# ml-jku/LaM-SLidE

Measured on AMD Instinct MI355X. Metric: sampled trajectories/sec (50-step ODE) + decoded-coord L2 vs ref, MD17, higher is better.
Workload: dtype bf16; 1 GPU; md17_bench; tail=False, ln_fuse=True, T=30, L=256, C=32, D=512, H=16, depth=4, sampler=ODE, state_updates=50, batch_per_gpu=32, global_batch=32, parallelism=batch-shard x1, 1 gather to rank 0 per step, noise_elem_stride_per_rank=7864320, kernels=general, trajectories_per_pass=32

## Files before the change

lam_slide_amd/csrc/host_launch.hip.h:

```cpp
#pragma once
#include <atomic>
#include <type_traits>

#include "host_common.hip.h"

namespace {

struct HeadArgs {
    float *x, *out;
    const float *h, *shift, *scale;
    int mod_stride;
    const float *Wo, *bo;
    int n, C, tpt, do_step;
    StepUpdate u;
};

#ifdef LSL_EXPERIMENTS
constexpr bool lsl_experiments = true;
template <int NE, int VEC>
bool launch_head_experiment(const HeadArgs &, hipStream_t);
template <class Epi>
bool launch_gemm_experiment(int, const GemmArgs &, const Epi &, hipStream_t, bool);
#else
constexpr bool lsl_experiments = false;
template <int NE, int VEC>
bool launch_head_experiment(const HeadArgs &, hipStream_t) { return false; }
template <class Epi>
bool launch_gemm_experiment(int, const GemmArgs &, const Epi &, hipStream_t, bool) { return false; }
#endif

int env_int(const char *name, int dflt) {
    const char *e = getenv(name);
    return e ? atoi(e) : dflt;
}
int tune_int(const char *name, int dflt) { return lsl_experiments ? env_int(name, dflt) : dflt; }

int device_cus() {
    static std::atomic<int> cache[64];
    int dev = 0;
    if (hipGetDevice(&dev) != hipSuccess) return 256;
    int n = cache[dev & 63].load(std::memory_order_relaxed);
    if (n > 0) return n;
    n = 256;
    (void)hipDeviceGetAttribute(&n, hipDeviceAttributeMultiprocessorCount, dev);
    if (n <= 0) n = 256;
    cache[dev & 63].store(n, std::memory_order_relaxed);
    return n;
}

constexpr size_t LDS_BUDGET = 160 * 1024;


template <int NE, int VEC>
void launch_ln_mod_t(u16 *a, const float *h, const float *shift, const float *scale, int stride, int n, int tpt, hipStream_t st) {
    if constexpr (NE % 4 == 0) {
        static const int persist = tune_int("LSL_LN_PERSIST", 16);
        if (persist > 0) {
            const int grid = std::min((n + 3) / 4, device_cus() * persist);
            static const int nt = (tune_int("LSL_NT", 3) >> 3) & 1;
            hipLaunchKernelGGL((k_ln_modulate_v4<NE>), dim3(grid), dim3(256), 0, st, a, h, shift, scale, stride, n, tpt, nt);
            return;
        }
    }
    hipLaunchKernelGGL((k_ln_modulate<NE, VEC>), dim3((n + 3) / 4), dim3(256), 0, st, a, h, shift, scale, stride, n, tpt);
}
template <int NE, int VEC>
void launch_ln_inplace_t(float *h, int n, float eps, hipStream_t st) {
    hipLaunchKernelGGL((k_ln_inplace<NE, VEC>), dim3((n + 3) / 4), dim3(256), 0, st, h, n, eps);
}
template <int NE, int VEC>
void launch_head_mfma(const HeadArgs &a, hipStream_t st, Profiler *pr = nullptr) {
    if (launch_head_experiment<NE, VEC>(a, st)) return;
    auto kern = k_head_step_mfma<NE, VEC>;
    const size_t lds = head_mfma_lds_bytes<NE>(a.C <= 32);
    LSL_ALLOW_LDS(kern, head_mfma_lds_bytes<NE>(false));
    static const int per_cu = tune_int("LSL_HEAD_PER_CU", 2);
    const int wgs = device_cus() * (per_cu >= 2 && 2 * lds <= LDS_BUDGET ? 2 : 1);
    if (pr) pr->label(4, "k_head_step_mfma<%d, %d> (%s, %d per CU)", NE, VEC, a.C <= 32 ? "one slab" : "cycled slabs", wgs / device_cus());
    hipLaunchKernelGGL(kern, dim3(std::min((a.n + HEAD_TOK - 1) / HEAD_TOK, wgs)), dim3(256), lds, st, a.x, a.out, a.h, a.shift, a.scale, a.mod_stride,
                       a.Wo, a.bo, a.n, a.C, a.tpt, a.do_step, a.u);
}
void launch_state_affine(float *x, unsigned long long n, const StepUpdate &u, hipStream_t st) {
    hipLaunchKernelGGL(k_state_affine, dim3((unsigned)std::min<unsigned long long>((n + 255) / 256, 2048)), dim3(256), 0, st, x, n, u);
}

#define DISPATCH_D(D, FN, ...)                          \
    switch ((D) / 64) {                                 \
        case 1: FN<1, 1>(__VA_ARGS__); break;           \
        case 2: FN<2, 2>(__VA_ARGS__); break;           \
        case 3: FN<3, 1>(__VA_ARGS__); break;           \
        case 4: FN<4, 2>(__VA_ARGS__); break;           \
        case 5: FN<5, 1>(__VA_ARGS__); break;           \
        case 6: FN<6, 2>(__VA_ARGS__); break;           \
        case 7: FN<7, 1>(__VA_ARGS__); break;           \
        default: FN<8, 2>(__VA_ARGS__); break;          \
    }

bool embed_stats_ok(int C, int D) { return C <= 32 && D % 256 == 0 && D <= 512; }
template <int MODE>
int launch_embed(float *out, const float *in, const float *W, const float *b, const float *b2, const float *me,
                 const int64_t *mask, const float *base, int n, int C, int D, hipStream_t st, float2 *stats = nullptr, int npad = 0,
                 Profiler *pr = nullptr) {
    if (C > 32 && C % 8 == 0 && C <= 128 && D % 32 == 0) {
        const int tpw = 3, ngrp = (D / 32 + tpw - 1) / tpw;
        const long units = (long)((n + 31) / 32) * ngrp;
        const dim3 g((unsigned)((units + 3) / 4));
        if (pr) pr->label(5, "k_embed_mfma<%d, %d> (32-token tiles)", MODE, C / 8);
        switch (C / 8) {
#define LSL_EMB_CASE(CK) case CK: hipLaunchKernelGGL((k_embed_mfma<MODE, CK>), g, dim3(256), 0, st, out, in, W, b, b2, me, mask, base, n, C, D, tpw); return 0;
            LSL_EMB_CASE(5) LSL_EMB_CASE(6) LSL_EMB_CASE(7) LSL_EMB_CASE(8) LSL_EMB_CASE(9) LSL_EMB_CASE(10) LSL_EMB_CASE(11) LSL_EMB_CASE(12)
            LSL_EMB_CASE(13) LSL_EMB_CASE(14) LSL_EMB_CASE(15) LSL_EMB_CASE(16)
#undef LSL_EMB_CASE
        }
    }
    int tok = EMB_TOK;
    static const int stage = tune_int("LSL_EMBED_LDS", 1);
    const bool w_lds = stage && C == 32 && D % 4 == 0 && D <= 512;
    if (w_lds)
        while (tok > 16 && (n + tok - 1) / tok < 2 * device_cus()) tok /= 2;
    const dim3 grid(std::min((n + tok - 1) / tok, 2 * device_cus())), blk(256);
    const bool with_stats = stats && MODE == 1 && C <= 32 && embed_stats_ok(C, D);
    if (pr)
        pr->label(5, "k_embed<%d, %d, %d%s> (%d-token tiles%s)", C <= 32 ? 32 : C <= 64 ? 64 : C <= 96 ? 96 : 128, MODE, C <= 32 ? 4 : C <= 96 ? 2 : 1,
                  with_stats ? ", true" : "", tok, w_lds ? ", weights through LDS" : (C & 3) ? ", scalar weight loads" : "");
    if (C <= 32) {
        const size_t lds = w_lds ? embed_w_lds_bytes<32, 4>(D) : 0;
        if (with_stats) {
            auto kern = k_embed<32, 1, 4, true>;
            LSL_ALLOW_LDS(kern, (embed_w_lds_bytes<32, 4>(512)));
            hipLaunchKernelGGL(kern, grid, blk, lds, st, out, in, W, b, b2, me, mask, base, n, C, D, w_lds ? 1 : 0, tok, stats, npad);
            return 0;
        }
        auto kern = k_embed<32, MODE, 4>;
        LSL_ALLOW_LDS(kern, (embed_w_lds_bytes<32, 4>(512)));
        hipLaunchKernelGGL(kern, grid, blk, lds, st, out, in, W, b, b2, me, mask, base, n, C, D, w_lds ? 1 : 0, tok, (float2 *)nullptr, 0);
    } else if (C <= 64) hipLaunchKernelGGL((k_embed<64, MODE, 2>), grid, blk, 0, st, out, in, W, b, b2, me, mask, base, n, C, D, 0, tok, (float2 *)nullptr, 0);
    else if (C <= 96) hipLaunchKernelGGL((k_embed<96, MODE, 2>), grid, blk, 0, st, out, in, W, b, b2, me, mask, base, n, C, D, 0, tok, (float2 *)nullptr, 0);
    else hipLaunchKernelGGL((k_embed<128, MODE, 1>), grid, blk, 0, st, out, in, W, b, b2, me, mask, base, n, C, D, 0, tok, (float2 *)nullptr, 0);
    return 0;
}

template <int BF, int BT, int NWF, int NWT, int BK, int NS, bool PERSIST, class Epi>
void launch_gemm_glds(const GemmArgs &g, const Epi &epi, hipStream_t st) {
    auto kern = k_gemm_glds<BF, BT, NWF, NWT, BK, NS, PERSIST, Epi>;
    const size_t lds = GemmCfg<BF, BT, NWF, NWT, BK, NS, PERSIST, Epi>::lds_bytes + (Epi::lds_bias ? (size_t)((g.F + BF - 1) / BF) * BF * 4 : 0);
    LSL_ALLOW_LDS(kern, LDS_BUDGET);
    const int tiles = ((g.N + BT - 1) / BT) * ((g.F + BF - 1) / BF);
    int grid = tiles;
    if (PERSIST) {
        const int per_cu = (int)std::max<size_t>(1, LDS_BUDGET / lds);
        grid = device_cus() * per_cu;
        grid -= grid % 8;
        if (grid > tiles) grid = tiles;
    }
    hipLaunchKernelGGL(kern, dim3(grid), dim3(NWF * NWT * 64), lds, st, g, epi);
}

}

#ifdef LSL_EXPERIMENTS
#include "host_launch_experiments.hip.h"
#endif

namespace {

template <class Fn>
bool with_linear1_ts_instance(int hdp, int D, Fn &&fn) {
#define X(H, K) if (hdp == H && D == K) return fn(ic<H>{}, ic<K>{}), true;
    LSL_LIN1_TS_INSTANCES(X)
#undef X
    return false;
}
template <int HDP, int K, int NW = 8, bool LNF = false>
void launch_linear1_ts_t(const Lin1Args &a, hipStream_t st) {
    using C = Lin1Cfg<HDP, K, NW>;
    const int ntile = (a.N + C::TT - 1) / C::TT, nb = a.F / 32;
    const long units = (long)ntile * nb;
    int grid = (int)std::min<long>(device_cus(), units / 2);
    Lin1Args b = a;
    static const int align = tune_int("LSL_LIN1_ALIGN", 1);
    const int wpt = std::min(device_cus() / ntile, nb / 2);
    b.wpt = align && wpt >= 2 ? wpt : 0;
    if (b.wpt) grid = b.wpt * ntile;
    lsl_lin1_launch(HDP, K, NW, LNF, b, grid, LNF ? C::lds_bytes_lnf(a.F) : C::lds_bytes(a.F), st);
}
int linear1_ts_waves(int D, int N) {
    static const int nw4_max = tune_int("LSL_LIN1_NW4_MAX", 10240);
    return D == 512 && N <= nw4_max ? 4 : 8;
}
bool linear1_ts_ok(int hdp, int D, int F1, int HHD, int N) {
    static const int on = tune_int("LSL_LIN1_TS", 1);
    if (!on || F1 % 64 != 0 || HHD % 64 != 0 || N < 1) return false;
    size_t lds = 0;
    return with_linear1_ts_instance(hdp, D, [&](auto h, auto k) { lds = Lin1Cfg<decltype(h)::value, decltype(k)::value, 8>::lds_bytes(F1); }) && lds <= LDS_BUDGET;
}
int ln_fuse_env() {
    static const int v = env_int("LSL_LN_FUSE", -1);
    return v;
}
bool linear1_lnf_ok(int hdp, int D, int F1, int HHD, int N, int tpt, int mod_stride) {
    if (ln_fuse_env() == 0 || !linear1_ts_ok(hdp, D, F1, HHD, N)) return false;
    size_t lds = 0;
    int min_tpt = 0;
    with_linear1_ts_instance(hdp, D, [&](auto h, auto k) {
        using C = Lin1Cfg<decltype(h)::value, decltype(k)::value, 8>;
        lds = C::lds_bytes_lnf(F1);
        min_tpt = C::LN_SLOTS >= 3 ? C::TT / 2 : C::TT;
    });
    return (mod_stride == 0 || tpt >= min_tpt) && lds <= LDS_BUDGET;
}
void launch_linear1_ts(int hdp, int D, int waves, bool lnf, const Lin1Args &a, hipStream_t st) {
    with_linear1_ts_instance(hdp, D, [&](auto h, auto k) {
        constexpr int H = decltype(h)::value, K = decltype(k)::value;
        if (lnf) return launch_linear1_ts_t<H, K, 8, true>(a, st);
        if constexpr (K == 512) {
            if (waves == 4) return launch_linear1_ts_t<H, K, 4>(a, st);
        }
        launch_linear1_ts_t<H, K, 8>(a, st);
    });
}

#define LSL_LIN2_WS_INSTANCES(X) X(1536, 3, 3) X(1280, 4, 4) X(768, 3, 3) X(384, 3, 3)
template <class Fn>
bool with_linear2_ws_instance(int K2, Fn &&fn) {
#define X(K, NCH, NS) if (K2 == K) return fn(ic<K>{}, ic<NCH>{}, ic<NS>{}), true;
    LSL_LIN2_WS_INSTANCES(X)
#undef X
    return false;
}
bool linear2_ws_shape_ok(int D, int K2) {
    static const int on = env_int("LSL_LIN2_WS", 1);
    return on && D % 128 == 0 && D <= 512 && with_linear2_ws_instance(K2, [](auto, auto, auto) {});
}
struct Lin2Grid {
    int slices, rpx, gate_rows;
};
Lin2Grid linear2_ws_grid(int F, int N, int tpt, bool shared) {
    const int slices = F / 128, cus = device_cus(), NBLK = (N + 31) / 32;
    int rpx = std::max(1, cus / (8 * slices));
    while (rpx > 1 && 8 * rpx > NBLK) --rpx;
    const int ranges = 8 * rpx, max_blocks = (NBLK + ranges - 1) / ranges + 1;
    return {slices, rpx, shared ? 1 : (max_blocks * 32 + tpt - 1) / tpt + 1};
}
int linear2_ws_max_gate_rows(int K2) {
    int rows = 0;
    with_linear2_ws_instance(K2, [&](auto k, auto nch, auto ns) { rows = Lin2Cfg<decltype(k)::value, decltype(nch)::value, decltype(ns)::value, true>::max_gate_rows; });
    return rows;
}
template <int K, int NCH, int NS, bool LNS>
void launch_linear2_ws_t(const Lin2Args &a, hipStream_t st) {
    using C = Lin2Cfg<K, NCH, NS, true>;
    auto kern = k_linear2_ws<K, NCH, NS, true, LNS>;
    LSL_ALLOW_LDS(kern, LDS_BUDGET);
    hipLaunchKernelGGL(kern, dim3(8 * a.slices * a.rpx), dim3(512), C::lds_bytes(a.gate_rows), st, a);
}
void launch_linear2_ws(int K2, const Lin2Args &a, hipStream_t st) {
    with_linear2_ws_instance(K2, [&](auto k, auto nch, auto ns) {
        constexpr int K = decltype(k)::value, NCH = decltype(nch)::value, NS = decltype(ns)::value;
        if (a.stats) launch_linear2_ws_t<K, NCH, NS, true>(a, st);
        else launch_linear2_ws_t<K, NCH, NS, false>(a, st);
    });
}

int tail_env() {
    static const int v = env_int("LSL_TAIL", -1);
    return v;
}
bool tail_shape_ok(int D, int HHD, int M) {
    return tail_env() != 0 && D == 256 && HHD == 256 && M % 64 == 0 && M >= 64 && TailCfg<256, 256>::lds_bytes(M) <= LDS_BUDGET;
}
size_t tail_stream_bytes(const lsl_model *m) { return TailCfg<256, 256>::stream_bytes(m->d.mlp_dim); }
void launch_tail(const TailArgs &a, hipStream_t st) {
    using C = TailCfg<256, 256>;
    auto kern = k_tail<256, 256>;
// ... 211 lines not shown
```

lam_slide_amd/csrc/k_small.hip.h:

```cpp
#pragma once
#include "common.hip.h"
#include "k_small_frag.hip.h"

__global__ void k_rope_table(float2 *tab, int n_pos, int hd, int hdp, float theta) {
    const int i = blockIdx.x * blockDim.x + threadIdx.x;
    const int half = hdp / 2;
    if (i >= n_pos * half) return;
    const int p = i / half, j = i % half;
    float2 v = make_float2(1.0f, 0.0f);
    if (2 * j < hd) {
        const double omega = 1.0 / pow((double)theta, (double)(2 * j) / (double)hd);
        const double ang = (double)p * omega;
        v = make_float2((float)cos(ang), (float)sin(ang));
    }
    tab[i] = v;
}

struct RopeScaledJobs {
    float4 *out[16];
    const float *scale[16];
    int n_pos[16];
    float *sq_bound[16];
    int n_jobs;
};
__global__ void k_rope_scaled(RopeScaledJobs jobs, int hd, int hdp, float theta) {
    const int job = blockIdx.y;
    if (job >= jobs.n_jobs) return;
    if (blockIdx.x == 0 && threadIdx.x == 0 && jobs.sq_bound[job]) {
        float mx = 0.0f;
        for (int d = 0; d < hd; ++d) mx = fmaxf(mx, jobs.scale[job][d] * jobs.scale[job][d]);
        *jobs.sq_bound[job] = mx * (float)hd;
    }
    const int half = hdp / 2, i = blockIdx.x * blockDim.x + threadIdx.x;
    if (i >= jobs.n_pos[job] * half) return;
    const int p = i / half, j = i % half;
    float c = 1.0f, sn = 0.0f;
    if (2 * j < hd) {
        const double omega = 1.0 / pow((double)theta, (double)(2 * j) / (double)hd);
        const double ang = (double)p * omega;
        c = (float)cos(ang);
        sn = (float)sin(ang);
    }
    const float s0 = jobs.scale[job][2 * j], s1 = jobs.scale[job][2 * j + 1];
    jobs.out[job][i] = make_float4(c * s0, sn * s1, sn * s0, c * s1);
}

__global__ void k_planes_to_rows(u16 *rows, const u16 *planes, int n, int npad, int heads3, int hdp) {
    const long i = (long)blockIdx.x * blockDim.x + threadIdx.x;
    const int cph = hdp / 8;
    if (i >= (long)n * heads3 * cph) return;
    const int c = (int)(i % cph), p = (int)((i / cph) % heads3);
    const long tok = (i / cph) / heads3;
    *reinterpret_cast<u32x4 *>(rows + (tok * heads3 + p) * hdp + 8 * c) = *reinterpret_cast<const u32x4 *>(planes + ((long)p * npad + tok) * hdp + 8 * c);
}

__global__ void k_time_features(float *out, const float *t_ptr, float t_scalar, const float *freqs, int rows) {
    const int i = blockIdx.x * blockDim.x + threadIdx.x;
    if (i >= rows * 128) return;
    const int b = i >> 7, k = i & 127;
    const float t = 1000.0f * (t_ptr ? t_ptr[b] : t_scalar);
    const float a = t * freqs[k];
    out[b * 256 + k] = cosf(a);
    out[b * 256 + 128 + k] = sinf(a);
}

struct StepTimes {
    float t[48];
};
__global__ void k_time_features_steps(float *out, StepTimes st, int n_steps, int rows_per_step, const float *freqs) {
    const int i = blockIdx.x * blockDim.x + threadIdx.x;
    if (i >= n_steps * rows_per_step * 128) return;
    const int row = i >> 7, k = i & 127;
    const float a = 1000.0f * st.t[row / rows_per_step] * freqs[k];
    out[row * 256 + k] = cosf(a);
    out[row * 256 + 128 + k] = sinf(a);
}

template <bool PRE_SILU, bool POST_SILU>
__global__ void __launch_bounds__(256) k_dense_rows(float *out, const float *in, const float *W, const float *bias,
                                                    const float *add, int rows, int I, int O, int add_stride, int add_mod) {
    const int lane = threadIdx.x & 63;
    const int o = blockIdx.x * 4 + (threadIdx.x >> 6);
    if (o >= O) return;
    float w[8];
#pragma unroll
    for (int k = 0; k < 8; ++k) {
        const int i = lane + 64 * k;
        w[k] = i < I ? W[(size_t)o * I + i] : 0.0f;
    }
    const float bo = bias[o];
    const int rpb = (rows + (int)gridDim.y - 1) / (int)gridDim.y, b_hi = min(rows, ((int)blockIdx.y + 1) * rpb);
    for (int b0 = (int)blockIdx.y * rpb; b0 < b_hi; b0 += 4) {
        float v[4][8];
#pragma unroll
        for (int r = 0; r < 4; ++r) {
            const int b = b0 + r;
            if (b >= b_hi) break;
#pragma unroll
            for (int k = 0; k < 8; ++k) {
                const int i = lane + 64 * k;
                v[r][k] = i < I ? in[(size_t)b * I + i] : 0.0f;
            }
        }
#pragma unroll
        for (int r = 0; r < 4; ++r) {
            const int b = b0 + r;
            if (b >= b_hi) break;
            float s = 0.0f;
#pragma unroll
            for (int k = 0; k < 8; ++k) {
                const int i = lane + 64 * k;
                if (i < I) s = fmaf(w[k], PRE_SILU ? silu(v[r][k]) : v[r][k], s);
            }
            s = wave_sum(s);
            if (lane == 0) dense_store<POST_SILU>(out, s, bo, add, b, o, O, add_stride, add_mod);
        }
    }
}

template <bool PRE_SILU, bool POST_SILU>
__global__ void __launch_bounds__(256) k_dense_tiled(float *out, const float *in, const float *W, const float *bias,
                                                     const float *add, int rows, int I, int O, int add_stride, int add_mod) {
    __shared__ __attribute__((aligned(16))) float As[16][64 + 4];
    __shared__ __attribute__((aligned(16))) float Ws[16][64 + 4];
    const int tid = threadIdx.x, tx = tid & 15, ty = tid >> 4;
    const int r0 = blockIdx.y * 64, o0 = blockIdx.x * 64;
    float acc[4][4];
#pragma unroll
    for (int i = 0; i < 4; ++i)
#pragma unroll
        for (int j = 0; j < 4; ++j) acc[i][j] = 0.0f;
    const int lr = tid >> 2, lk = (tid & 3) * 4;
    for (int k0 = 0; k0 < I; k0 += 16) {
        float4 a = make_float4(0.f, 0.f, 0.f, 0.f), w = make_float4(0.f, 0.f, 0.f, 0.f);
        if (r0 + lr < rows && k0 + lk < I) a = *reinterpret_cast<const float4 *>(in + (size_t)(r0 + lr) * I + k0 + lk);
        if (o0 + lr < O && k0 + lk < I) w = *reinterpret_cast<const float4 *>(W + (size_t)(o0 + lr) * I + k0 + lk);
        if (PRE_SILU) a = make_float4(silu(a.x), silu(a.y), silu(a.z), silu(a.w));
        __syncthreads();
        As[lk][lr] = a.x; As[lk + 1][lr] = a.y; As[lk + 2][lr] = a.z; As[lk + 3][lr] = a.w;
        Ws[lk][lr] = w.x; Ws[lk + 1][lr] = w.y; Ws[lk + 2][lr] = w.z; Ws[lk + 3][lr] = w.w;
        __syncthreads();
#pragma unroll
        for (int k = 0; k < 16; ++k) {
            const float4 av = *reinterpret_cast<const float4 *>(&As[k][4 * ty]);
            const float4 wv = *reinterpret_cast<const float4 *>(&Ws[k][4 * tx]);
            const float ar[4] = {av.x, av.y, av.z, av.w}, wr[4] = {wv.x, wv.y, wv.z, wv.w};
#pragma unroll
            for (int i = 0; i < 4; ++i)
#pragma unroll
                for (int j = 0; j < 4; ++j) acc[i][j] = fmaf(ar[i], wr[j], acc[i][j]);
        }
    }
#pragma unroll
// ... 4 lines not shown
        for (int j = 0; j < 4; ++j) {
            const int o = o0 + 4 * tx + j;
            if (o >= O) continue;
            dense_store<POST_SILU>(out, acc[i][j], bias[o], add, b, o, O, add_stride, add_mod);
        }
    }
}

template <bool PRE_SILU, bool POST_SILU, int KQ>
__global__ void __launch_bounds__(256) k_dense_mfma(float *out, const float *in, const float *W, const float *bias, const float *add,
                                                    int rows, int I, int O, int add_stride, int add_mod) {
    __shared__ PartTile Ps[4];
    const int tid = threadIdx.x, lane = tid & 63, wave = tid >> 6, r = lane & 31, hf = lane >> 5;
    const int r0 = blockIdx.y * 32, o0 = blockIdx.x * 32;
    const float *ap = in + (size_t)min(r0 + r, rows - 1) * I + wave * KQ + 4 * hf;
    const float *wp = W + (size_t)min(o0 + r, O - 1) * I + wave * KQ + 4 * hf;
    float4 a[KQ / 8], w[KQ / 8];
#pragma unroll
    for (int j = 0; j < KQ / 8; ++j) {
        a[j] = *reinterpret_cast<const float4 *>(ap + 8 * j);
        w[j] = *reinterpret_cast<const float4 *>(wp + 8 * j);
    }
    f32x16 acc = f32x16_zero();
#pragma unroll
    for (int j = 0; j < KQ / 8; ++j) {
        float4 av = a[j];
        if (PRE_SILU) av = make_float4(silu(av.x), silu(av.y), silu(av.z), silu(av.w));
        acc = mfma32_f32x4(av, w[j], acc);
    }
#pragma unroll
    for (int e = 0; e < 16; ++e) Ps[wave][acc_row(e, hf)][r] = acc[e];
    __syncthreads();
#pragma unroll
    for (int q = 0; q < 4; ++q) {
        const int idx = tid + 256 * q, row = idx >> 5, col = idx & 31, b = r0 + row, o = o0 + col;
        if (b >= rows || o >= O) continue;
        dense_store<POST_SILU>(out, part_sum(Ps, row, col), bias[o], add, b, o, O, add_stride, add_mod);
    }
}

constexpr int EMB_TOK = 64;
template <int CMAX, int ND>
constexpr size_t embed_w_lds_bytes(int D) { return (size_t)(D / ND) * (ND * CMAX / 4 + 1) * 16; }
template <int CMAX, int MODE, int ND, bool STATS = false>
__global__ void __launch_bounds__(256) k_embed(float *out, const float *in, const float *W, const float *bias,
                                               const float *bias2, const float *mask_emb, const int64_t *mask,
                                               const float *base, int N, int C, int D, int w_lds, int tok, float2 *stats = nullptr, int npad = 0) {
    __shared__ __attribute__((aligned(16))) float xs[EMB_TOK][CMAX];
    extern __shared__ __attribute__((aligned(16))) float4 embed_w_lds[];
    const int n_tiles = (N + tok - 1) / tok;
    const int DQ = D / ND, groups = DQ >= 256 ? 1 : 256 / DQ;
    for (int dq = threadIdx.x % (DQ < 256 ? DQ : 256), trip = 0; trip < (DQ + 255) / 256; dq += 256, ++trip) {
        const int tg = DQ >= 256 ? 0 : threadIdx.x / DQ, d = ND * dq;
        const bool active = tg < groups && dq < DQ;
        float w[ND][CMAX];
        if (w_lds) {
            constexpr int PIECES = ND * CMAX / 4;
            const int n4 = D * CMAX / 4;
            const float4 *W4 = reinterpret_cast<const float4 *>(W);
#pragma unroll 8
            for (int i = threadIdx.x; i < n4; i += 256) embed_w_lds[(i / PIECES) * (PIECES + 1) + (i % PIECES)] = W4[i];
            __syncthreads();
#pragma unroll
            for (int j = 0; j < ND; ++j)
#pragma unroll
                for (int c = 0; c < CMAX; c += 4) {
                    const float4 w4 = active ? embed_w_lds[dq * (PIECES + 1) + (j * CMAX + c) / 4] : make_float4(0.f, 0.f, 0.f, 0.f);
                    w[j][c] = w4.x; w[j][c + 1] = w4.y; w[j][c + 2] = w4.z; w[j][c + 3] = w4.w;
                }
        } else if ((C & 3) == 0) {
#pragma unroll
            for (int j = 0; j < ND; ++j)
#pragma unroll
                for (int c = 0; c < CMAX; c += 4) {
                    const float4 w4 = (active && c < C) ? *reinterpret_cast<const float4 *>(W + (size_t)(d + j) * C + c) : make_float4(0.f, 0.f, 0.f, 0.f);
                    w[j][c] = w4.x; w[j][c + 1] = w4.y; w[j][c + 2] = w4.z; w[j][c + 3] = w4.w;
                }
        } else {
#pragma unroll
            for (int j = 0; j < ND; ++j)
#pragma unroll
                for (int c = 0; c < CMAX; ++c) w[j][c] = (active && c < C) ? W[(size_t)(d + j) * C + c] : 0.0f;
        }
        float b0[ND];
#pragma unroll
        for (int j = 0; j < ND; ++j) b0[j] = (MODE == 0 && active) ? bias[d + j] + bias2[d + j] : 0.0f;
        for (int tile = blockIdx.x; tile < n_tiles; tile += gridDim.x) {
            const int n0 = tile * tok;
            const int ntok = min(tok, N - n0);
            __syncthreads();
            for (int i = threadIdx.x; i < tok * CMAX; i += 256) {
                const int tkn = i / CMAX, c = i % CMAX;
                xs[tkn][c] = (tkn < ntok && c < C) ? in[(size_t)(n0 + tkn) * C + c] : 0.0f;
            }
            __syncthreads();
            if (!active) continue;
            constexpr int PF = 4;
            for (int t0 = tg; t0 < ntok; t0 += PF * groups) {
                float add[PF][ND];
#pragma unroll
                for (int u = 0; u < PF; ++u) {
                    const int tkn = min(t0 + u * groups, ntok - 1);
                    const size_t row = (size_t)(n0 + tkn) * D + d;
                    if (MODE == 0) {
                        const float *me = mask_emb + (mask[n0 + tkn] != 0 ? D : 0) + d;
#pragma unroll
                        for (int j = 0; j < ND; ++j) add[u][j] = b0[j] + me[j];
                    } else {
#pragma unroll
                        for (int j = 0; j < ND; ++j) add[u][j] = base[row + j];
                    }
                }
#pragma unroll
                for (int u = 0; u < PF; ++u) {
                    const int tkn = t0 + u * groups;
                    if (tkn >= ntok) break;
                    const size_t row = (size_t)(n0 + tkn) * D + d;
                    float acc[ND];
#pragma unroll
                    for (int j = 0; j < ND; ++j) acc[j] = 0.0f;
#pragma unroll
                    for (int c = 0; c < CMAX; c += 4) {
                        const float4 xv = *reinterpret_cast<const float4 *>(&xs[tkn][c]);
#pragma unroll
                        for (int j = 0; j < ND; ++j) acc[j] = fmaf(xv.x, w[j][c], acc[j]);
#pragma unroll
                        for (int j = 0; j < ND; ++j) acc[j] = fmaf(xv.y, w[j][c + 1], acc[j]);
#pragma unroll
                        for (int j = 0; j < ND; ++j) acc[j] = fmaf(xv.z, w[j][c + 2], acc[j]);
#pragma unroll
                        for (int j = 0; j < ND; ++j) acc[j] = fmaf(xv.w, w[j][c + 3], acc[j]);
                    }
#pragma unroll
                    for (int j = 0; j < ND; ++j) acc[j] = acc[j] + add[u][j];
#pragma unroll
                    for (int j = 0; j < ND; ++j) out[row + j] = acc[j];
                    if constexpr (STATS) {
                        float s = 0.0f;
#pragma unroll
                        for (int j = 0; j < ND; ++j) s += acc[j];
                        const float mean = wave_sum_dpp(s) * (1.0f / (64.0f * ND));
                        float q = 0.0f;
#pragma unroll
                        for (int j = 0; j < ND; ++j) q = fmaf(acc[j] - mean, acc[j] - mean, q);
                        const float m2 = wave_sum_dpp(q);
                        if ((threadIdx.x & 63) == 0) stats[(size_t)(dq >> 6) * npad + n0 + tkn] = make_float2(mean, m2);
                    }
                }
            }
        }
    }
}

template <int MODE, int CK>
__global__ void __launch_bounds__(256) k_embed_mfma(float *out, const float *in, const float *W, const float *bias, const float *bias2,
                                                    const float *mask_emb, const int64_t *mask, const float *base, int N, int C, int D,
                                                    int tiles_per_wave) {
    const int lane = threadIdx.x & 63, wave = threadIdx.x >> 6, r = lane & 31, hf = lane >> 5;
    const int nft = D / 32, ngrp = (nft + tiles_per_wave - 1) / tiles_per_wave;
    const long unit = (long)blockIdx.x * 4 + wave;
    const long n_units = (long)((N + 31) / 32) * ngrp;
    if (unit >= n_units) return;
    const int n0 = (int)(unit / ngrp) * 32, ft0 = (int)(unit % ngrp) * tiles_per_wave;
    float4 a[CK];
    {
        const float *ap = in + (size_t)min(n0 + r, N - 1) * C + 4 * hf;
#pragma unroll
        for (int j = 0; j < CK; ++j) a[j] = *reinterpret_cast<const float4 *>(ap + 8 * j);
    }
    for (int ft = ft0; ft < min(ft0 + tiles_per_wave, nft); ++ft) {
        const int d0 = ft * 32;
        float4 w[CK];
        const float *wp = W + (size_t)(d0 + r) * C + 4 * hf;
#pragma unroll
        for (int j = 0; j < CK; ++j) w[j] = *reinterpret_cast<const float4 *>(wp + 8 * j);
        float addv[16];
#pragma unroll
        for (int e = 0; e < 16; ++e) {
            const int n = min(n0 + acc_row(e, hf), N - 1);
            if (MODE == 0) addv[e] = mask_emb[(mask[n] != 0 ? D : 0) + d0 + r];
            else addv[e] = base[(size_t)n * D + d0 + r];
        }
        const float b0 = MODE == 0 ? bias[d0 + r] + bias2[d0 + r] : 0.0f;
        f32x16 acc = f32x16_zero();
#pragma unroll
        for (int j = 0; j < CK; ++j) acc = mfma32_f32x4(a[j], w[j], acc);
#pragma unroll
        for (int e = 0; e < 16; ++e) {
            const int n = n0 + acc_row(e, hf);
            if (n < N) out[(size_t)n * D + d0 + r] = MODE == 0 ? acc[e] + (b0 + addv[e]) : acc[e] + addv[e];
        }
    }
}

template <int NE, int VEC>
__device__ __forceinline__ int row_col(int lane, int e) { return VEC == 2 ? 2 * lane + 128 * (e >> 1) + (e & 1) : lane + 64 * e; }

template <int NE, int VEC>
__device__ __forceinline__ void row_load(const float *row, int lane, float (&v)[NE]) {
    if (VEC == 2) {
#pragma unroll
        for (int k = 0; k < NE / 2; ++k) {
            const float2 t = *reinterpret_cast<const float2 *>(row + 2 * lane + 128 * k);
            v[2 * k] = t.x;
            v[2 * k + 1] = t.y;
        }
    } else {
#pragma unroll
        for (int k = 0; k < NE; ++k) v[k] = row[lane + 64 * k];
    }
}
template <int NE, bool DPP = false>
__device__ __forceinline__ void row_stats(const float (&v)[NE], float eps, float &mean, float &rstd) {
    constexpr float invD = 1.0f / (float)(NE * 64);
    float s = 0.0f;
#pragma unroll
    for (int k = 0; k < NE; ++k) s += v[k];
    mean = (DPP ? wave_sum_dpp(s) : wave_sum(s)) * invD;
    float q = 0.0f;
#pragma unroll
    for (int k = 0; k < NE; ++k) {
        const float a = v[k] - mean;
        q += a * a;
    }
    rstd = rsqrtf((DPP ? wave_sum_dpp(q) : wave_sum(q)) * invD + eps);
}

template <int NE, int VEC>
__global__ void __launch_bounds__(256) k_ln_inplace(float *h, int N, float eps) {
    const int lane = threadIdx.x & 63;
    const int n = blockIdx.x * 4 + (threadIdx.x >> 6);
    if (n >= N) return;
    constexpr int D = NE * 64;
    float *row = h + (size_t)n * D;
    float v[NE];
    row_load<NE, VEC>(row, lane, v);
    float mean, rstd;
    row_stats<NE>(v, eps, mean, rstd);
#pragma unroll
    for (int k = 0; k < NE; ++k) row[row_col<NE, VEC>(lane, k)] = (v[k] - mean) * rstd;
}

template <int NE, int VEC>
__global__ void __launch_bounds__(256) k_ln_modulate(u16 *a, const float *h, const float *shift, const float *scale,
                                                     int mod_stride, int N, int tokens_per_traj) {
    const int lane = threadIdx.x & 63;
    const int n = blockIdx.x * 4 + (threadIdx.x >> 6);
    if (n >= N) return;
    constexpr int D = NE * 64;
    float v[NE];
    row_load<NE, VEC>(h + (size_t)n * D, lane, v);
    float mean, rstd;
    row_stats<NE>(v, 1e-6f, mean, rstd);
    const size_t mo = (size_t)(n / tokens_per_traj) * mod_stride;
    u16 *arow = a + (size_t)n * D;
    if (VEC == 2) {
#pragma unroll
        for (int k = 0; k < NE / 2; ++k) {
            const int d = 2 * lane + 128 * k;
            const float2 sc = *reinterpret_cast<const float2 *>(scale + mo + d);
            const float2 sf = *reinterpret_cast<const float2 *>(shift + mo + d);
            *reinterpret_cast<unsigned *>(arow + d) = pack2(ln_mod_scale(v[2 * k], mean, rstd, sc.x, sf.x), ln_mod_scale(v[2 * k + 1], mean, rstd, sc.y, sf.y));
        }
    } else {
#pragma unroll
        for (int k = 0; k < NE; ++k) {
            const int d = lane + 64 * k;
            arow[d] = f2bf(ln_mod_scale(v[k], mean, rstd, scale[mo + d], shift[mo + d]));
        }
    }
}

template <int NE>
__global__ void __launch_bounds__(256) k_ln_modulate_v4(u16 *a, const float *h, const float *shift, const float *scale, int mod_stride,
                                                        int N, int tokens_per_traj, int nt) {
    static_assert(NE % 4 == 0, "D must be a multiple of 256");
    constexpr int D = NE * 64, Q = NE / 4;
    constexpr float invD = 1.0f / (float)D;
    const int lane = threadIdx.x & 63;
    const int stride = gridDim.x * 4;
    int n = blockIdx.x * 4 + (threadIdx.x >> 6);
    if (n >= N) return;
    float4 v[Q], vn[Q];
#pragma unroll
    for (int k = 0; k < Q; ++k) v[k] = *reinterpret_cast<const float4 *>(h + (size_t)n * D + 4 * lane + 256 * k);
    for (; n < N; n += stride) {
        const int nn = n + stride < N ? n + stride : n;
#pragma unroll
        for (int k = 0; k < Q; ++k) vn[k] = *reinterpret_cast<const float4 *>(h + (size_t)nn * D + 4 * lane + 256 * k);
        float s = 0.0f;
#pragma unroll
        for (int k = 0; k < Q; ++k) s += (v[k].x + v[k].y) + (v[k].z + v[k].w);
        const float mean = wave_sum(s) * invD;
        float q = 0.0f;
#pragma unroll
        for (int k = 0; k < Q; ++k) {
            const float dx = v[k].x - mean, dy = v[k].y - mean, dz = v[k].z - mean, dw = v[k].w - mean;
            q += (dx * dx + dy * dy) + (dz * dz + dw * dw);
        }
        const float rstd = rsqrtf(wave_sum(q) * invD + 1e-6f);
        const size_t mo = (size_t)(n / tokens_per_traj) * mod_stride;
#pragma unroll
        for (int k = 0; k < Q; ++k) {
            const int d = 4 * lane + 256 * k;
            const float4 sc = *reinterpret_cast<const float4 *>(scale + mo + d);
            const float4 sf = *reinterpret_cast<const float4 *>(shift + mo + d);
// ... 201 lines not shown
```

lam_slide_amd/csrc/k_small_frag.hip.h:

```cpp
#pragma once
#include "common.hip.h"

typedef __attribute__((ext_vector_type(4))) float f32x4v;

__device__ __forceinline__ f32x16 mfma32_f32x4(float4 a, float4 b, f32x16 c) {
    c = __builtin_amdgcn_mfma_f32_32x32x2f32(a.x, b.x, c, 0, 0, 0);
    c = __builtin_amdgcn_mfma_f32_32x32x2f32(a.y, b.y, c, 0, 0, 0);
    c = __builtin_amdgcn_mfma_f32_32x32x2f32(a.z, b.z, c, 0, 0, 0);
    return __builtin_amdgcn_mfma_f32_32x32x2f32(a.w, b.w, c, 0, 0, 0);
}
__device__ __forceinline__ f32x4v mfma16_f32x4(float4 a, float4 b, f32x4v c) {
    c = __builtin_amdgcn_mfma_f32_16x16x4f32(a.x, b.x, c, 0, 0, 0);
    c = __builtin_amdgcn_mfma_f32_16x16x4f32(a.y, b.y, c, 0, 0, 0);
    c = __builtin_amdgcn_mfma_f32_16x16x4f32(a.z, b.z, c, 0, 0, 0);
    return __builtin_amdgcn_mfma_f32_16x16x4f32(a.w, b.w, c, 0, 0, 0);
}
__device__ __forceinline__ f32x16 f32x16_zero() {
    f32x16 z;
#pragma unroll
    for (int e = 0; e < 16; ++e) z[e] = 0.0f;
    return z;
}

typedef float PartTile[32][33];
constexpr int PART_FLOATS = 4 * 32 * 33;
template <class P>
__device__ __forceinline__ void part_scatter(P &Ps, int wave, int r, int hf, const f32x16 &acc) {
#pragma unroll
    for (int e = 0; e < 16; ++e) Ps[wave][acc_row(e, hf)][r] = acc[e];
}
template <class P>
__device__ __forceinline__ float part_sum(const P &Ps, int row, int col) {
    return ((Ps[0][row][col] + Ps[1][row][col]) + Ps[2][row][col]) + Ps[3][row][col];
}

template <bool POST_SILU>
__device__ __forceinline__ void dense_store(float *out, float s, float bias_o, const float *add, int b, int o, int O, int add_stride, int add_mod) {
    s += bias_o;
    if (add) s += add[(size_t)(add_mod ? b % add_mod : b) * add_stride + o];
    if (POST_SILU) s = silu(s);
    out[(size_t)b * O + o] = s;
}

__device__ __forceinline__ float ln_mod(float v, float mean, float rstd, float sc1, float shift) { return (v - mean) * rstd * sc1 + shift; }
__device__ __forceinline__ float ln_mod_scale(float v, float mean, float rstd, float scale, float shift) { return (v - mean) * rstd * (1.0f + scale) + shift; }

template <class T>
__device__ __forceinline__ T block_tree_sum(T *red, T v) {
    red[threadIdx.x] = v;
    __syncthreads();
    for (int o = 128; o > 0; o >>= 1) {
        if ((int)threadIdx.x < o) red[threadIdx.x] += red[threadIdx.x + o];
        __syncthreads();
    }
    return red[0];
}

__device__ __forceinline__ void philox4x32_10(unsigned (&c)[4], unsigned k0, unsigned k1) {
#pragma unroll
    for (int r = 0; r < 10; ++r) {
        const unsigned long long p0 = (unsigned long long)0xD2511F53u * c[0];
        const unsigned long long p1 = (unsigned long long)0xCD9E8D57u * c[2];
        const unsigned n0 = (unsigned)(p1 >> 32) ^ c[1] ^ k0;
        const unsigned n1 = (unsigned)p1;
        const unsigned n2 = (unsigned)(p0 >> 32) ^ c[3] ^ k1;
        const unsigned n3 = (unsigned)p0;
        c[0] = n0; c[1] = n1; c[2] = n2; c[3] = n3;
        k0 += 0x9E3779B9u;
        k1 += 0xBB67AE85u;
    }
}
__device__ __forceinline__ float philox_normal(unsigned long long seed, unsigned step, unsigned long long elem) {
    const unsigned long long blk = elem >> 2;
    unsigned c[4] = {(unsigned)blk, (unsigned)(blk >> 32), step, 0u};
    philox4x32_10(c, (unsigned)seed, (unsigned)(seed >> 32));
    const int pair = (int)(elem & 2);
    const float u1 = ((float)c[pair] + 1.0f) * 2.3283064365386963e-10f;
    const float u2 = (float)c[pair + 1] * 2.3283064365386963e-10f;
    const float rad = sqrtf(-2.0f * __logf(u1));
    float sn, cs;
    __sincosf(6.283185307179586f * u2, &sn, &cs);
    return (elem & 1) ? rad * sn : rad * cs;
}

struct StepUpdate {
    const float *noise;
    float *trace;
    const float *saved;
    float *save_out;
    unsigned long long seed, elem_offset;
    float ax, am, aw, as;
    unsigned step;
};
__device__ __forceinline__ float step_noise(const float *noise, unsigned long long seed, unsigned step, unsigned long long elem_offset, size_t e) {
    return noise ? noise[e] : philox_normal(seed, step, elem_offset + e);
}
template <bool NET>
__device__ __forceinline__ float step_value(const StepUpdate &u, size_t e, float x_old, float m) {
    float xn = NET ? u.ax * x_old + u.am * m : u.ax * x_old;
    if (u.aw != 0.0f) xn += u.aw * step_noise(u.noise, u.seed, u.step, u.elem_offset, e);
    if (u.saved) xn += u.as * u.saved[e];
    return xn;
}
template <bool NET>
__device__ __forceinline__ void step_apply(const StepUpdate &u, float *x, size_t e, float x_old, float m) {
    const float xn = step_value<NET>(u, e, x_old, m);
    x[e] = xn;
    if (u.trace) u.trace[e] = xn;
    if (u.save_out) u.save_out[e] = xn;
}
```

Baseline: 56.67 trajectories/s.

## Add streaming embed kernel with async LDS prefetch ring for base rows

Adds k_embed_stream, a persistent embed kernel that keeps the 32-wide weight slice in registers. It double-buffers input tiles and prefetches the base rows into an 8-deep LDS ring through direct global-to-LDS DMA, using vmcnt waits and custom barriers. The goal is to hide global-memory latency for the base-row add and input loads in the bandwidth-bound embed step. It is used for MODE 1 with D of 256 or 512 when there are enough tokens per CU. The hand-tuned vmcnt counting is fragile and could produce wrong results if the wait counts are off.

```diff
diff --git a/lam_slide_amd/csrc/host_launch.hip.h b/lam_slide_amd/csrc/host_launch.hip.h
--- a/lam_slide_amd/csrc/host_launch.hip.h
+++ b/lam_slide_amd/csrc/host_launch.hip.h
@@ -49,6 +49,7 @@
 }
 
 constexpr size_t LDS_BUDGET = 160 * 1024;
+constexpr int STREAM_MIN_TOKENS_PER_CU = 256;
 
 
 template <int NE, int VEC>
@@ -120,6 +121,23 @@
         while (tok > 16 && (n + tok - 1) / tok < 2 * device_cus()) tok /= 2;
     const dim3 grid(std::min((n + tok - 1) / tok, 2 * device_cus())), blk(256);
     const bool with_stats = stats && MODE == 1 && C <= 32 && embed_stats_ok(C, D);
+    if constexpr (MODE == 1) {
+        const int stream = env_int("LSL_EMBED_STREAM", 1);
+        if (w_lds && (D == 256 || D == 512) && n <= (1 << 30) && (stream >= 2 || (stream == 1 && n >= STREAM_MIN_TOKENS_PER_CU * device_cus()))) {
+            const dim3 sgrid(std::min((n + EMB_TOK - 1) / EMB_TOK, 2 * device_cus()));
+            const size_t lds = embed_stream_lds_bytes(D);
+            if (pr) pr->label(5, "k_embed_stream<%d%s> (64-token tiles, base rows %d tokens ahead)", D, with_stats ? ", true" : ", false", EMBS_RING);
+#define LSL_EMBS_CASE(DD, ST)                                                                                          \
+    if (D == DD && with_stats == ST) {                                                                                 \
+        auto kern = k_embed_stream<DD, ST>;                                                                            \
+        LSL_ALLOW_LDS(kern, embed_stream_lds_bytes(DD));                                                               \
+        hipLaunchKernelGGL(kern, sgrid, blk, lds, st, out, in, W, base, n, with_stats ? stats : (float2 *)nullptr, npad); \
+        return 0;                                                                                                      \
+    }
+            LSL_EMBS_CASE(256, false) LSL_EMBS_CASE(256, true) LSL_EMBS_CASE(512, false) LSL_EMBS_CASE(512, true)
+#undef LSL_EMBS_CASE
+        }
+    }
     if (pr)
         pr->label(5, "k_embed<%d, %d, %d%s> (%d-token tiles%s)", C <= 32 ? 32 : C <= 64 ? 64 : C <= 96 ? 96 : 128, MODE, C <= 32 ? 4 : C <= 96 ? 2 : 1,
                   with_stats ? ", true" : "", tok, w_lds ? ", weights through LDS" : (C & 3) ? ", scalar weight loads" : "");
diff --git a/lam_slide_amd/csrc/k_small.hip.h b/lam_slide_amd/csrc/k_small.hip.h
--- a/lam_slide_amd/csrc/k_small.hip.h
+++ b/lam_slide_amd/csrc/k_small.hip.h
@@ -1,4 +1,6 @@
 #pragma once
+#include <type_traits>
+
 #include "common.hip.h"
 #include "k_small_frag.hip.h"
 
@@ -309,6 +311,115 @@
     }
 }
 
+constexpr int EMBS_RING = 8;
+constexpr size_t EMBS_XS_BYTES = 2 * EMB_TOK * 32 * 4, EMBS_LDS_BYTES = EMBS_XS_BYTES + EMBS_RING * 4096;
+constexpr size_t embed_stream_lds_bytes(int D) { return embed_w_lds_bytes<32, 4>(D) > EMBS_LDS_BYTES ? embed_w_lds_bytes<32, 4>(D) : EMBS_LDS_BYTES; }
+template <int D, bool STATS>
+__global__ void __launch_bounds__(256) k_embed_stream(float *out, const float *in, const float *W, const float *base, int N, float2 *stats, int npad) {
+    constexpr int CMAX = 32, ND = 4, PIECES = ND * CMAX / 4, R = EMBS_RING, DQ = D / ND, GROUPS = 256 / DQ, TPT = EMB_TOK / GROUPS;
+    constexpr int KS = STATS ? 2 : 1;
+    static_assert(DQ == 64 || DQ == 128, "a token row is one or two waves");
+    static_assert(TPT % R == 0 && TPT > R, "the ring divides a thread's tokens of a tile; the input requests are older than the last token's piece");
+    static_assert(KS + (R - 1) * (1 + KS) <= 63, "vmcnt");
+    extern __shared__ __attribute__((aligned(16))) float4 embed_w_lds[];
+    const unsigned lds0 = (unsigned)(size_t)(LDS_PTR(char))(embed_w_lds);
+    const int n_tiles = (N + EMB_TOK - 1) / EMB_TOK;
+    const int lane = threadIdx.x & 63, wave = __builtin_amdgcn_readfirstlane((int)threadIdx.x >> 6);
+    const int dq = threadIdx.x % DQ, tg = wave / (DQ / 64), d = ND * dq;
+    float w[ND][CMAX];
+    {
+        const float4 *W4 = reinterpret_cast<const float4 *>(W);
+#pragma unroll 8
+        for (int i = threadIdx.x; i < D * CMAX / 4; i += 256) embed_w_lds[(i / PIECES) * (PIECES + 1) + (i % PIECES)] = W4[i];
+        __syncthreads();
+#pragma unroll
+        for (int j = 0; j < ND; ++j)
+#pragma unroll
+            for (int c = 0; c < CMAX; c += 4) {
+                const float4 w4 = embed_w_lds[dq * (PIECES + 1) + (j * CMAX + c) / 4];
+                w[j][c] = w4.x; w[j][c + 1] = w4.y; w[j][c + 2] = w4.z; w[j][c + 3] = w4.w;
+            }
+        __syncthreads();
+    }
+    auto request_in = [&](int tile, int buf) __attribute__((always_inline)) {
+        const char *src = uni_ptr(reinterpret_cast<const char *>(in + (size_t)min(tile * EMB_TOK, N - 1) * CMAX));
+#pragma unroll
+        for (int q = 0; q < 2; ++q) {
+            const int piece = 2 * wave + q, tkn = 8 * piece + (lane >> 3);
+            const int rel = min(tile * EMB_TOK + tkn, N - 1) - min(tile * EMB_TOK, N - 1);
+            lds_dma16((unsigned)rel * 128u + 16u * (lane & 7), src, __builtin_amdgcn_readfirstlane(lds0 + (unsigned)buf * 8192u + 1024u * piece));
+        }
+    };
+    auto request_base = [&](int n, int u) __attribute__((always_inline)) {
+        const char *src = uni_ptr(reinterpret_cast<const char *>(base + (size_t)min(n, N - 1) * D + 256 * (wave % (DQ / 64))));
+        lds_dma16(16u * lane, src, __builtin_amdgcn_readfirstlane(lds0 + (unsigned)EMBS_XS_BYTES + 4096u * u + 1024u * wave));
+    };
+    const float4 *ring = embed_w_lds + EMBS_XS_BYTES / 16 + threadIdx.x;
+    int tile = blockIdx.x, buf = 0;
+    request_in(tile, 0);
+#pragma unroll
+    for (int u = 0; u < R; ++u) request_base(tile * EMB_TOK + tg + GROUPS * u, u);
+    wait_vmcnt<R>();
+    stream_barrier();
+    bool fresh = true;
+    for (; tile < n_tiles; tile += gridDim.x, buf ^= 1) {
+        const int n0 = tile * EMB_TOK, next = tile + (int)gridDim.x;
+        request_in(next, buf ^ 1);
+        const float(*xs)[CMAX] = reinterpret_cast<const float(*)[CMAX]>(embed_w_lds + buf * 512);
+        auto walk = [&](auto full_c) __attribute__((always_inline)) {
+            constexpr bool FULL = decltype(full_c)::value;
+#pragma unroll 1
+            for (int k0 = 0; k0 < TPT; k0 += R) {
+                const int nb = (k0 + R < TPT ? n0 + GROUPS * (k0 + R) : next * EMB_TOK + GROUPS * (k0 + R - TPT)) + tg;
+#pragma unroll
+                for (int u = 0; u < R; ++u) {
+                    const int tkn = tg + GROUPS * (k0 + u);
+                    float acc[ND];
+#pragma unroll
+                    for (int j = 0; j < ND; ++j) acc[j] = 0.0f;
+#pragma unroll
+                    for (int c = 0; c < CMAX; c += 4) {
+                        const float4 xv = *reinterpret_cast<const float4 *>(&xs[tkn][c]);
+#pragma unroll
+                        for (int j = 0; j < ND; ++j) acc[j] = fmaf(xv.x, w[j][c], acc[j]);
+#pragma unroll
+                        for (int j = 0; j < ND; ++j) acc[j] = fmaf(xv.y, w[j][c + 1], acc[j]);
+#pragma unroll
+                        for (int j = 0; j < ND; ++j) acc[j] = fmaf(xv.z, w[j][c + 2], acc[j]);
+#pragma unroll
+                        for (int j = 0; j < ND; ++j) acc[j] = fmaf(xv.w, w[j][c + 3], acc[j]);
+                    }
+                    if (FULL && !fresh) wait_vmcnt<KS + (R - 1) * (1 + KS)>();
+                    else wait_vmcnt<R - 1>();
+                    const float4 add = ring[256 * u];
+                    acc[0] = acc[0] + add.x; acc[1] = acc[1] + add.y; acc[2] = acc[2] + add.z; acc[3] = acc[3] + add.w;
+                    asm volatile("" : "+v"(acc[0]), "+v"(acc[1]), "+v"(acc[2]), "+v"(acc[3]));
+                    request_base(nb + GROUPS * u, u);
+                    if (FULL || n0 + tkn < N) {
+                        *reinterpret_cast<float4 *>(out + (size_t)(n0 + tkn) * D + d) = make_float4(acc[0], acc[1], acc[2], acc[3]);
+                        if constexpr (STATS) {
+                            float s = 0.0f;
+#pragma unroll
+                            for (int j = 0; j < ND; ++j) s += acc[j];
+                            const float mean = wave_sum_dpp(s) * (1.0f / (64.0f * ND));
+                            float q = 0.0f;
+#pragma unroll
+                            for (int j = 0; j < ND; ++j) q = fmaf(acc[j] - mean, acc[j] - mean, q);
+                            const float m2 = wave_sum_dpp(q);
+                            if (lane == 0) stats[(size_t)(dq >> 6) * npad + n0 + tkn] = make_float2(mean, m2);
+                        }
+                    }
+                }
+                fresh = false;
+            }
+        };
+        if (n0 + EMB_TOK <= N) walk(std::true_type{});
+        else walk(std::false_type{});
+        stream_barrier();
+    }
+    wait_vmcnt<0>();
+}
+
 template <int MODE, int CK>
 __global__ void __launch_bounds__(256) k_embed_mfma(float *out, const float *in, const float *W, const float *bias, const float *bias2,
                                                     const float *mask_emb, const int64_t *mask, const float *base, int N, int C, int D,
diff --git a/lam_slide_amd/csrc/k_small_frag.hip.h b/lam_slide_amd/csrc/k_small_frag.hip.h
--- a/lam_slide_amd/csrc/k_small_frag.hip.h
+++ b/lam_slide_amd/csrc/k_small_frag.hip.h
@@ -32,6 +32,12 @@
 template <class P>
 __device__ __forceinline__ float part_sum(const P &Ps, int row, int col) {
     return ((Ps[0][row][col] + Ps[1][row][col]) + Ps[2][row][col]) + Ps[3][row][col];
+}
+
+__device__ __forceinline__ void stream_barrier() {
+    asm volatile("s_waitcnt lgkmcnt(0)" ::: "memory");
+    __builtin_amdgcn_s_barrier();
+    asm volatile("" ::: "memory");
 }
 
 template <bool POST_SILU>
```

Result: no change. 56.74 trajectories/s, median of 2 (+0.1%).
